# hyunjik11/GPT

Measured on AMD Instinct MI355X. Metric: SGLD steps/sec (kin40k, n_feat=500/dim, r=5), higher is better.
Workload: dtype f64

## Files before the change

gpt_amd/csrc/chain.hip:

```cpp
#include "device_util.h"

namespace gpt {

constexpr int kChainBufs = 1;
constexpr int kChainDMax = 8;
constexpr int kChainTPW8 = 1;
constexpr int kChainTasks = 2;
constexpr int kChainG = 2;
constexpr int kChainQPL = 4;
constexpr int kChainQP = 64 * kChainQPL;
constexpr int kChainRun = 64;
constexpr int kChainRunS = 72;
constexpr int kChainQS = 264;

constexpr int kChainMMax = 256;

GPT_HD constexpr int chain_scratch_dbl(int r, bool own_x1) {
  const int s0a = 7 * 4 * r * r, s0b = 64 * 8;
  return (s0a > s0b ? s0a : s0b) + (own_x1 ? 7 : 2) * r * r + 3 * r * r + r;
}
GPT_HD constexpr int al16c(int x) { return (x + 15) & ~15; }

template <int R, int G, int WV = kChainDMax>
struct ChainLds {
  static constexpr int DRG = kChainDMax * R * G;
  static constexpr int TS = 2 * (DRG + G);
  static constexpr int NTMAX = kChainQPL * G;
  static constexpr int o_IT = 0;
  static constexpr int o_w = al16c(o_IT + 4 * kChainQP * kChainDMax);
  static constexpr int o_y = al16c(o_w + 8 * kChainQP);
  static constexpr int o_temp = al16c(o_y + 8 * kChainMMax);
  static constexpr int o_fp = al16c(o_temp + 8 * 2 * TS);
  static constexpr int o_gwp = al16c(o_fp + 8 * kChainQPL * G);
  static constexpr int o_misc = al16c(o_gwp + 8 * NTMAX * 64);
  static constexpr int o_touch = al16c(o_misc + 8 * 16);
  static constexpr int o_un = al16c(o_touch + 256);
  static constexpr int L_dbl = G * kChainQS + WV * G * R * kChainRunS;
  static constexpr bool own_x1 = WV == kChainDMax;
  static constexpr int x_dbl = chain_scratch_dbl(R, own_x1);
  static constexpr int o_tab = al16c(o_un + 8 * (L_dbl > x_dbl * WV ? L_dbl : x_dbl * WV));
  static constexpr bool tab = WV == kChainDMax;
  static constexpr int bytes = al16c(o_tab + (tab ? 8 * 64 : 0));
};

#ifndef CHAIN_TIMELINE
#define CHAIN_TIMELINE 2
#endif

#ifndef CHAIN_SSTAMP
#define CHAIN_SSTAMP 0
#endif
#ifndef CHAIN_STAMPS
#define CHAIN_STAMPS CHAIN_SSTAMP
#endif
#define CHAIN_FENCE() do {} while (0)
#ifndef CHAIN_PRIO
#define CHAIN_PRIO 2
#endif
#define CHAIN_SETPRIO(hi_upper)                                                             \
  do {                                                                                      \
    if (CHAIN_PRIO) {                                                                       \
      if ((k >= 4) == (hi_upper)) __builtin_amdgcn_s_setprio(1);                            \
      else __builtin_amdgcn_s_setprio(0);                                                   \
    }                                                                                       \
  } while (0)
#if !CHAIN_STAMPS
#define CSTAMP(slot) CHAIN_FENCE()
#endif
#if CHAIN_TIMELINE
#define TSTAMP_ANY(i)                                                                       \
  do {                                                                                      \
    if (P.tline && tid == 0 && (i) < kTimelineSteps + 2) {                                  \
      long long* ts_ = P.tline + (size_t)blockIdx.x * kTimeline + 2 * (i);                  \
      ts_[0] = (long long)__builtin_amdgcn_s_memrealtime();                                \
      ts_[1] = (long long)__builtin_amdgcn_s_memtime();                                    \
    }                                                                                       \
  } while (0)
#else
#define TSTAMP_ANY(i) do {} while (0)
#endif
#if CHAIN_TIMELINE == 1
#define TSTAMP(i) TSTAMP_ANY(i)
#else
#define TSTAMP(i) do {} while (0)
#endif
#if CHAIN_STAMPS
#define CSTAMP(slot)                                                                        \
  do {                                                                                      \
    if (P.stamps && tid == 0)                                                               \
      P.stamps[(size_t)blockIdx.x * kStamps + (slot)] = (long long)__builtin_amdgcn_s_memtime(); \
  } while (0)
#endif

#if CHAIN_STAMPS
#define LSTAMP(slot)                                                                        \
  do {                                                                                      \
    if (P.stamps && g0 == 20 && lane == 0 && (k == 0 || k == 4))                            \
      P.stamps[(size_t)(gridDim.x + blockIdx.x) * kStamps + (k ? 8 : 0) + (slot)] =         \
          (long long)__builtin_amdgcn_s_memtime();                                         \
  } while (0)
#else
#define LSTAMP(slot) CHAIN_FENCE()
#endif

#define SSTAMP(slot)                                                                        \
  do {                                                                                      \
    if ((slot) == 4) CHAIN_SETPRIO(false);        \
    if ((slot) == 7) CHAIN_SETPRIO(true);        \
    if (CHAIN_SSTAMP && P.stamps && lane == 0 && (k == 0 || k == 4))                                        \
      P.stamps[(size_t)((2 + (slot) / 8) * gridDim.x + blockIdx.x) * kStamps + (k ? 8 : 0) + \
               (slot) % 8] = (long long)__builtin_amdgcn_s_memtime();                       \
  } while (0)

template <int J>
__device__ __forceinline__ bool row_in(int jj, int j, int n) {
  return (J >= 2 && jj < J / 2) || j < n;
}

__device__ __forceinline__ void lds_barrier() {
  asm volatile("s_waitcnt lgkmcnt(0)\n\ts_barrier" ::: "memory");
}

template <int R, int J, int G, int WV>
__global__ __launch_bounds__(64 * WV, WV == 4 ? 2 : 1) void chain_kernel(StepParams P,
                                                                const ChainDesc* chains,
                                                                const long long* __restrict__ tbase,
                                                                int t_local, int nsteps) {
  extern __shared__ __attribute__((aligned(16))) unsigned char smem[];
  __shared__ __attribute__((aligned(16))) double pbuf[kChainBufs * WV * G * 64 * J];
  __shared__ __attribute__((aligned(16))) int ibuf[2 * kChainMMax];
  const ChainDesc* Cp = chains + blockIdx.x;
  const int tid = threadIdx.x, lane = tid & 63, k = uni(tid >> 6);
  const int n = P.n, D = P.D, Q = P.Q, m = P.m, NTH = 64 * D;
  using L = ChainLds<R, G, WV>;
  const int NCH = (Q + 63) / 64, NT = NCH * G;
  int* IT_l = (int*)(smem + L::o_IT);
  double* w_l = (double*)(smem + L::o_w);
  int* idx_l = ibuf;
  double* y_l = (double*)(smem + L::o_y);
  double* temp_l = (double*)(smem + L::o_temp);
  double* fp_l = (double*)(smem + L::o_fp);
  double* gwp_l = (double*)(smem + L::o_gwp);
  double* misc = (double*)(smem + L::o_misc);
  int* flag = (int*)(misc + 8);
  double* wVr = (double*)(smem + L::o_un);
  double* X = (double*)(smem + L::o_un) + k * L::x_dbl;
  double* xi_l = X;
  double* pw0 = pbuf + k * (kChainBufs * G * 64 * J);
  [[maybe_unused]] double* bscr = wVr + G * kChainQS + k * G * R * kChainRunS;

  TSTAMP_ANY(0);
#if CHAIN_TIMELINE
  if (P.tline && tid == 0) {
    long long* ts_ = P.tline + (size_t)blockIdx.x * kTimeline + kTimeline - 2;
    ts_[0] = (long long)__builtin_amdgcn_s_getreg((31 << 11) | 4);
    ts_[1] = (long long)__builtin_amdgcn_s_getreg((31 << 11) | 20);
  }
#endif
  const long long t0 = tbase[0] + t_local;
  if (t0 >= P.total_steps) return;
  if (__hip_atomic_load(Cp->status, __ATOMIC_RELAXED, __HIP_MEMORY_SCOPE_AGENT) != 0) return;
  CSTAMP(0);
  const long long tend = min(P.total_steps, t0 + (long long)nsteps);

  auto batch_at = [&](const int32_t* order, int ep_, int bb_, int& bt) -> const int32_t* {
    bt = min(m, P.N - bb_ * m);
    return order + (size_t)ep_ * P.N + (size_t)bb_ * m;
  };
  auto next_pos = [&](int& ep_, int& bb_) {
    if (++bb_ == P.nb) { bb_ = 0; ep_ ^= 1; }
  };
  long long t = t0;
  int ep, bb;
  {
    const int ee = (int)(t0 / P.nb);
    bb = (int)(t0 - (long long)ee * P.nb);
    ep = ee & 1;
  }
  int st_cd;
  long long st_slot;
  {
    const long long post0 = t0 - P.burnin_steps;
    long long cd;
    if (post0 < 0) {
      cd = P.store_every - 1 - post0;
      st_slot = 0;
    } else {
      const long long rem = (post0 + 1) % P.store_every;
      cd = rem ? P.store_every - rem : 0;
      st_slot = (post0 + 1 + cd) / P.store_every - 1;
    }
    st_cd = (int)min(cd, (long long)0x7fffffff);
  }
  int Bt;
  const int32_t* ord = batch_at(Cp->order, ep, bb, Bt);
  const long long koff = (long long)n * k, rstride = (long long)n * D;
  const double* phi_k = uni_ptr(Cp->phi) + koff;
  auto stage_rows = [&](const int (&rows)[G], int ln, double* pw) {
#pragma unroll
    for (int gg = 0; gg < G; ++gg) {
      const char* rb = (const char*)(phi_k + (long long)rows[gg] * rstride);
      __attribute__((address_space(3))) double* dst =
          (__attribute__((address_space(3))) double*)(pw + gg * 64 * J);
      if constexpr (J >= 2) {
#pragma unroll
        for (int s = 0; s < J / 2; ++s) {
          const unsigned o = min(16u * ln + 1024u * s, 8u * n - 16u);
          __builtin_amdgcn_global_load_lds((const __attribute__((address_space(1))) void*)(rb + o),
                                           (__attribute__((address_space(3))) void*)(dst + 128 * s),
                                           16, 0, 0);
        }
      } else {
#pragma unroll
        for (int s = 0; s < 2; ++s) {
          const unsigned o = min(4u * ln + 256u * s, 8u * n - 4u);
          __builtin_amdgcn_global_load_lds((const __attribute__((address_space(1))) void*)(rb + o),
                                           (__attribute__((address_space(3))) void*)(dst + 32 * s),
                                           4, 0, 0);
        }
      }
    }
  };
  auto stage = [&](int g0n, int ln, double* pw) {
    int rows[G];
#pragma unroll
    for (int gg = 0; gg < G; ++gg) rows[gg] = uni(idx_l[min(g0n + gg, Bt - 1)]);
    stage_rows(rows, ln, pw);
  };
  {
    int rows0[G];
#pragma unroll
    for (int gg = 0; gg < G; ++gg) rows0[gg] = gptr(ord)[min(gg, Bt - 1)];
    stage_rows(rows0, lane, pw0);
  }

  constexpr int DRG = L::DRG;
  {
    for (int o = tid; o < Q * kChainDMax; o += NTH) {
      const int kk = o / Q, q = o - kk * Q;
      IT_l[o] = kk < D ? (kk * R + gptr(P.I0)[q + Q * kk]) * G : DRG;
    }
    for (int o = tid; o < G; o += NTH) wVr[o * kChainQS + kChainQP] = 0.0;
    for (int o = tid; o < 2 * G; o += NTH) {
      temp_l[o / G * L::TS + DRG + o % G] = 1.0;
      temp_l[o / G * L::TS + 2 * DRG + G + o % G] = 1.0;
    }
    for (int o = tid; o < kChainQPL * G; o += NTH) fp_l[o] = 0.0;
  }
  if constexpr (L::tab) sincos_tab_fill((double*)(smem + L::o_tab), tid, NTH);
  for (int q = tid; q < Q; q += NTH) w_l[q] = gptr(Cp->w)[(size_t)(t0 & 1) * Q + q];
  if (tid == 0) flag[0] = 0;
  {
    const double* yv = Cp->y;
    int* i0_l = ibuf + ((int)t0 & 1) * kChainMMax;
    for (int i = tid; i < Bt; i += NTH) {
      const int row = gptr(ord)[i];
      i0_l[i] = row;
      y_l[i] = gptr(yv)[row];
    }
    if (t0 + 1 < tend) {
      int e1 = ep, b1 = bb, B1;
      next_pos(e1, b1);
      const int32_t* ord1 = batch_at(Cp->order, e1, b1, B1);
      int* i1_l = ibuf + ((int)(t0 + 1) & 1) * kChainMMax;
      for (int i = tid; i < B1; i += NTH) i1_l[i] = gptr(ord1)[i];
    }
  }
  double u[J][R];
  {
    const double* Ug = Cp->U + (size_t)n * R * k;
#pragma unroll
    for (int jj = 0; jj < J; ++jj) {
      const int j = lane + 64 * jj;
      const int jc = min(j, n - 1);
#pragma unroll
      for (int l = 0; l < R; ++l) {
        const double x = gptr(Ug + (size_t)n * l)[jc];
        u[jj][l] = j < n ? x : 0.0;
      }
    }
  }
  __syncthreads();
  CSTAMP(1);
  TSTAMP_ANY(1);



  constexpr int TPW = (J >= 8 && WV > 4) ? kChainTPW8 : kChainTasks;
  for (;;) {
  const int lane = lane_id(), tid = 64 * k + lane;
  idx_l = ibuf + ((int)t & 1) * kChainMMax;
  for (int o = tid; o < G; o += NTH) wVr[o * kChainQS + kChainQP] = 0.0;
  unsigned itp[TPW][kChainDMax / 4];
#pragma unroll
  for (int x = 0; x < TPW; ++x) {
    const int task = k + D * x;
    const int c = task < NT ? task % NCH : 0;
    const int qq = min(64 * c + lane, Q - 1);
#pragma unroll
    for (int h = 0; h < kChainDMax / 4; ++h) {
      unsigned v = 0;
#pragma unroll
      for (int b4 = 0; b4 < 4; ++b4) v |= (unsigned)IT_l[(4 * h + b4) * Q + qq] << (8 * b4);
      itp[x][h] = v;
    }
  }
  unsigned gq[4];
  {
    const int rl0 = min(lane >> 3, R - 1), rs0 = lane & 7;
    const int32_t* rq = P.runq + ((size_t)k * R + rl0) * kChainRun + rs0;
#pragma unroll
    for (int i = 0; i < 4; ++i)
      gq[i] = (unsigned)gptr(rq)[16 * i] | ((unsigned)gptr(rq)[16 * i + 8] << 16);
  }
  double acc[J][R];
#pragma unroll
  for (int jj = 0; jj < J; ++jj)
#pragma unroll
    for (int l = 0; l < R; ++l) acc[jj][l] = 0.0;
  double vsave[TPW], gw[TPW];
#pragma unroll
  for (int x = 0; x < TPW; ++x) { vsave[x] = 0.0; gw[x] = 0.0; }

  int slot = 0;
  for (int g0 = 0; g0 < Bt; g0 += G, slot ^= 1) {
    int ln = lane;
    asm volatile("" : "+v"(ln));
    LSTAMP(0);
    asm volatile("s_waitcnt vmcnt(0)" ::: "memory");
    LSTAMP(1);
    double* pw = pw0;
    double p[G][J];
#pragma unroll
    for (int gg = 0; gg < G; ++gg)
#pragma unroll
      for (int jj = 0; jj < J; ++jj)
        p[gg][jj] = pw[gg * 64 * J + ln + 64 * jj];
    asm volatile("s_waitcnt lgkmcnt(0)" ::: "memory");
    LSTAMP(2);
    double* tsl = temp_l + slot * L::TS;
    const int rl = min(ln >> 3, R - 1);
    {
      double v[G * R];
#pragma unroll
      for (int x = 0; x < G * R; ++x) v[x] = 0.0;
#pragma unroll
      for (int gg = 0; gg < G; ++gg)
#pragma unroll
        for (int jj = 0; jj < J; ++jj)
#pragma unroll
          for (int l = 0; l < R; ++l) v[gg * R + l] = fma(p[gg][jj], u[jj][l], v[gg * R + l]);
      obf_run<G * R, G * R>(v, ln);
      int vi;
      bool wr;
      obf_index<G * R>(ln, vi, wr);
      if (wr) {
        const int gg = vi / R, l = vi - gg * R;
        tsl[(k * R + l) * G + gg] = v[0];
        tsl[DRG + G + (k * R + l) * G + gg] = rcp_nr(v[0]);
      }
    }
    if (g0 + G < Bt) stage(g0 + G, ln, pw);
    LSTAMP(3);
    lds_barrier();
    LSTAMP(4);
#pragma unroll
    for (int x = 0; x < TPW; ++x) {
      const int task = k + D * x;
      if (task >= NT) break;
      const int gg = task / NCH, c = task - gg * NCH;
      const int q = 64 * c + ln;
      const bool ok = q < Q;
      const double wq = w_l[min(q, Q - 1)];
      double tv[kChainDMax];
#pragma unroll
      for (int kk = 0; kk < kChainDMax; ++kk)
        tv[kk] = tsl[((itp[x][kk >> 2] >> (8 * (kk & 3))) & 0xff) + gg];
      static_assert(kChainDMax == 8, "product tree below is written for 8 dimensions");
      const double V = ((tv[0] * tv[1]) * (tv[2] * tv[3])) * ((tv[4] * tv[5]) * (tv[6] * tv[7]));
      const double wV = ok ? wq * V : 0.0;
      if (ok) wVr[gg * kChainQS + q] = wV;
      vsave[x] = ok ? V : 0.0;
      const double fs = wave_sum(wV);
      if (lane == 0) fp_l[gg * kChainQPL + c] = fs;
    }
    LSTAMP(5);
    lds_barrier();
    LSTAMP(6);
    double res[G];
#pragma unroll
    for (int gg = 0; gg < G; ++gg) {
      double f = fp_l[gg * kChainQPL];
#pragma unroll
      for (int c = 1; c < kChainQPL; ++c) f += fp_l[gg * kChainQPL + c];
      res[gg] = (g0 + gg < Bt) ? y_l[g0 + gg] - f : 0.0;
    }
#pragma unroll
    for (int gg = 0; gg < G; ++gg) {
      const double* wr = wVr + gg * kChainQS;
      double a = wr[gq[0] & 0xffff];
#pragma unroll
      for (int i = 1; i < 8; ++i) a += wr[(gq[i >> 1] >> (16 * (i & 1))) & 0xffff];
      a = (group8_sum(a) * tsl[DRG + G + (k * R + rl) * G + gg]) * res[gg];
      double cc[R];
#pragma unroll
      for (int l = 0; l < R; ++l) cc[l] = readlane_d(a, 8 * l);
#pragma unroll
      for (int jj = 0; jj < J; ++jj) {
        const double pv = p[gg][jj];
#pragma unroll
        for (int l = 0; l < R; ++l) acc[jj][l] = fma(pv, cc[l], acc[jj][l]);
      }
    }
#pragma unroll
    for (int x = 0; x < TPW; ++x) {
      const int task = k + D * x;
      if (task >= NT) break;
      const int gg = task / NCH;
      double rr = res[0];
#pragma unroll
      for (int g2 = 1; g2 < G; ++g2) if (gg == g2) rr = res[g2];
      gw[x] = fma(vsave[x], rr, gw[x]);
    }
    LSTAMP(7);
  }
  CSTAMP(2);

  const ChainDesc* Cq = Cp;
  asm volatile("" : "+s"(Cq));
  ChainDesc C;
  {
    const auto* Cc = cptr(Cq);
    C.y = Cc->y; C.order = Cc->order; C.w = Cc->w; C.U = Cc->U;
    C.w_store = Cc->w_store; C.U_store = Cc->U_store; C.diag = Cc->diag; C.status = Cc->status;
    C.seed = Cc->seed; C.epsw = Cc->epsw; C.epsU = Cc->epsU; C.signal_var = Cc->signal_var;
    C.sigma_w = Cc->sigma_w;
  }
  int Nn = P.N;
  asm volatile("" : "+s"(Nn));
  const double cN = (double)Nn / (double)Bt;
  const bool store = st_cd == 0;
  const long long slot_s = store ? st_slot : 0;

#pragma unroll
  for (int x = 0; x < TPW; ++x) {
    const int task = k + D * x;
    if (task >= NT) break;
    gwp_l[task * 64 + lane] = gw[x];
  }
  SSTAMP(0);
  __syncthreads();
  SSTAMP(1);
  CHAIN_SETPRIO(true);
  int ep1 = ep, bb1 = bb, Bn = 0;
  next_pos(ep1, bb1);
  const int* idx_n = ibuf + ((int)(t + 1) & 1) * kChainMMax;
  double y_n = 0.0;
  if (t + 1 < tend) {
    Bn = min(m, P.N - bb1 * m);
    y_n = gptr(C.y)[idx_n[min(tid, Bn - 1)]];
  }
  {
    const double inv_sw2 = 1.0 / (C.sigma_w * C.sigma_w);
    const double sqe = sqrt(C.epsw);
    double gn2 = 0.0;
#pragma unroll 1
    for (int q = tid; q < Q; q += NTH) {
      const int c = q >> 6, ln = q & 63;
      double g = 0.0;
      for (int gg = 0; gg < G; ++gg) g += gwp_l[(gg * NCH + c) * 64 + ln];
      const double wq = w_l[q];
      const double gradw = cN * g / C.signal_var - wq * inv_sw2;
      double step = C.epsw * gradw / 2;
      step += sqe * normal_at(C.seed, (uint32_t)q, (uint32_t)t, kWNoise, 0);
      const double wn = wq + step;
      w_l[q] = wn;
      if (t + 1 == tend) gptr_w(C.w)[(size_t)((t + 1) & 1) * Q + q] = wn;
      if (store && C.w_store) gptr_w(C.w_store)[(size_t)slot_s * Q + q] = wn;
      gn2 = fma(gradw, gradw, gn2);
    }
    if (C.diag) {
      gn2 = wave_sum(gn2);
      if (lane == 0) misc[k] = gn2;
    }
  }
  SSTAMP(2);
  asm volatile("" : "+v"(y_n));
  if (t + 1 < tend) {
    y_l[min(tid, Bn - 1)] = y_n;
    for (int i = tid + NTH; i < Bn; i += NTH) y_l[i] = gptr(C.y)[idx_n[i]];
    int rows0[G];
#pragma unroll
    for (int gg = 0; gg < G; ++gg) rows0[gg] = uni(idx_n[min(gg, Bn - 1)]);
    stage_rows(rows0, lane, pw0);
    if (t + 2 < tend) {
      int ep2 = ep1, bb2 = bb1, B2;
      next_pos(ep2, bb2);
      const int32_t* ord2 = batch_at(C.order, ep2, bb2, B2);
#pragma unroll
      for (int x = 0; x < kChainMMax / 64; ++x) {
        const int c0 = 64 * k + x * NTH;
        if (c0 < B2)
          __builtin_amdgcn_global_load_lds(
              (const __attribute__((address_space(1))) void*)(ord2 + min(c0 + lane, B2 - 1)),
              (__attribute__((address_space(3))) void*)(idx_l + c0), 4, 0, 0);
      }
    }
  }
  CSTAMP(3);
  SSTAMP(3);

  const double cU = cN / C.signal_var;
  const double sq = sqrt(C.epsU);
  double gu2 = 0.0;
  {
    constexpr int NQJ = (J + 3) / 4;
    constexpr int NZ = J >= 4 ? 4 : 2;
    const int NQ = unoise_nq(n);
#pragma unroll 1
    for (int l = 0; l < R; ++l) {
#pragma unroll
      for (int q = 0; q < NQJ; ++q) {
        double z[4];
        if constexpr (L::tab)
          normal_quad_tab<NZ>(C.seed, (uint32_t)((l * NQ + q) * 64 + lane), (uint32_t)t, kUNoise,
                              (uint32_t)k, (const double*)(smem + L::o_tab), z);
        else
          normal_quad<NZ>(C.seed, (uint32_t)((l * NQ + q) * 64 + lane), (uint32_t)t, kUNoise,
                          (uint32_t)k, z);
#pragma unroll
        for (int i = 0; i < NZ; ++i)
          if (4 * q + i < J) xi_l[(4 * q + i) * 64 + lane] = z[i];
      }
#pragma unroll
      for (int L = 0; L < R; ++L) {
        if (l == L) {
          double xv[J];
#pragma unroll
          for (int jj = 0; jj < J; ++jj) xv[jj] = xi_l[jj * 64 + lane];
#pragma unroll
          for (int jj = 0; jj < J; ++jj) {
            const bool in = row_in<J>(jj, lane + 64 * jj, n);
            const double Gv = in ? acc[jj][L] * cU : 0.0;
            gu2 = fma(Gv, Gv, gu2);
            acc[jj][L] = in ? sq * Gv / 2 + xv[jj] : 0.0;
          }
        }
      }
    }
  }
  if (C.diag) {
    gu2 = wave_sum(gu2);
    if (lane == 0) C.diag[(size_t)t * (1 + D) + 1 + k] = sqrt(gu2);
  }
  CSTAMP(4);
  SSTAMP(4);
  {
    constexpr int NN = 2 * R;
    constexpr int S0 = (7 * NN * NN > 64 * 8) ? 7 * NN * NN : 64 * 8;
    constexpr bool kOwnX1 = L::own_x1;
    double* X0 = X;
    double* Ec = X + S0;
    double* X1 = kOwnX1 ? X + S0 : X0;
    double* Mg = X + S0 + (kOwnX1 ? 7 * R * R : NN * R);
    double* Ag = Mg + R * R;
    double* Sg = Ag + R * R;
    double* nr = Sg + R * R;
    wave_sync();
#pragma unroll
    for (int a = 0; a < R; ++a) {
      double v[R];
#pragma unroll
      for (int bb = 0; bb < R; ++bb) {
        double s0 = 0.0;
#pragma unroll
        for (int jj = 0; jj < J; ++jj) s0 = fma(u[jj][a], acc[jj][bb], s0);
        v[bb] = s0;
      }
      wave_sum_to_lds<R>(v, Mg + a * R);
    }
    wave_sync();
    SSTAMP(5);
#pragma unroll
    for (int bb = 0; bb < R; ++bb) {
      double ms[R];
#pragma unroll
      for (int a = 0; a < R; ++a) ms[a] = Mg[a * R + bb] + Mg[bb * R + a];
#pragma unroll
      for (int jj = 0; jj < J; ++jj) {
        double s = 0.0;
#pragma unroll
        for (int a = 0; a < R; ++a) s = fma(u[jj][a], ms[a], s);
        acc[jj][bb] = acc[jj][bb] - s / 2;
      }
    }
      CSTAMP(5);
      SSTAMP(6);
      {
#pragma unroll
        for (int a = 0; a < R; ++a) {
          double v[R];
#pragma unroll
          for (int bb = 0; bb < R; ++bb) {
            double s1 = 0.0;
            if (bb >= a)
#pragma unroll
              for (int jj = 0; jj < J; ++jj) s1 = fma(acc[jj][a], acc[jj][bb], s1);
            v[bb] = s1;
          }
          wave_sum_to_lds<R>(v, Sg + a * R);
        }
      }
      wave_sync();
      const double tt = sq;
      for (int o = lane; o < NN * NN; o += 64) {
        const int i = o / NN, j = o - i * NN;
        const int ia = i < R ? i : i - R, ja = j < R ? j : j - R;
        const double a = (Mg[ia * R + ja] - Mg[ja * R + ia]) / 2;
        double v;
        if (i < R) v = j < R ? a : -Sg[ia <= ja ? ia * R + ja : ja * R + ia];
        else v = j < R ? (ia == j ? 1.0 : 0.0) : a;
        X0[o] = tt * v;
        if (kOwnX1 && i < R && j < R) X1[ia * R + ja] = -tt * a;
        if (!kOwnX1 && i < R && j < R) Ag[ia * R + ja] = a;
      }
      wave_sync();
      long long* xst = (CHAIN_SSTAMP && P.stamps && k == 0)
                           ? P.stamps + (size_t)(4 * gridDim.x + blockIdx.x) * kStamps : nullptr;
      const bool bad = wave_expm<NN>(X0, xst);
      SSTAMP(7);
      if constexpr (!kOwnX1) {
        for (int o = lane; o < NN * R; o += 64) {
          const int a = o / R, l = o - a * R;
          Ec[o] = X0[NN * NN + a * NN + l];
        }
        wave_sync();
        for (int o = lane; o < R * R; o += 64) X1[o] = -tt * Ag[o];
        wave_sync();
      }
      wave_expm<R>(X1, xst ? xst + (size_t)gridDim.x * kStamps : nullptr);
      if (bad && lane == 0) flag[0] = 1;
      CSTAMP(6);
      SSTAMP(8);
      const double* mx = X1 + R * R;
      double* F = Mg;
      const double* El = kOwnX1 ? X0 + NN * NN : Ec;
      constexpr int ES = kOwnX1 ? NN : R;
      wave_sync();
      for (int o = lane; o < NN * R; o += 64) {
        const int a = o / R, l = o - a * R;
        double s = 0.0;
#pragma unroll
        for (int c2 = 0; c2 < R; ++c2) s = fma(El[a * ES + c2], mx[c2 * R + l], s);
        F[o] = s;
      }
      wave_sync();
      SSTAMP(9);
      {
        double Fh[R * R];
#pragma unroll
        for (int x = 0; x < R * R; ++x) Fh[x] = F[x];
#pragma unroll
        for (int jj = 0; jj < J; ++jj) {
          double o[R];
#pragma unroll
          for (int l = 0; l < R; ++l) o[l] = 0.0;
#pragma unroll
          for (int a = 0; a < R; ++a)
#pragma unroll
            for (int l = 0; l < R; ++l) o[l] = fma(u[jj][a], Fh[a * R + l], o[l]);
#pragma unroll
          for (int l = 0; l < R; ++l) u[jj][l] = o[l];
        }
      }
      SSTAMP(10);
      double nrm[R];
#pragma unroll
      for (int l = 0; l < R; ++l) nrm[l] = 0.0;
      {
        double Fh[R * R];
#pragma unroll
        for (int x = 0; x < R * R; ++x) Fh[x] = F[R * R + x];
#pragma unroll
        for (int jj = 0; jj < J; ++jj) {
#pragma unroll
          for (int a = 0; a < R; ++a)
#pragma unroll
            for (int l = 0; l < R; ++l) u[jj][l] = fma(acc[jj][a], Fh[a * R + l], u[jj][l]);
#pragma unroll
          for (int l = 0; l < R; ++l) nrm[l] = fma(u[jj][l], u[jj][l], nrm[l]);
        }
      }
      SSTAMP(11);
      wave_sum_to_lds<R>(nrm, nr);
      wave_sync();
      SSTAMP(12);
#pragma unroll
      for (int l = 0; l < R; ++l) {
        const double isc = 1.0 / sqrt(nr[l]);
#pragma unroll
        for (int jj = 0; jj < J; ++jj) u[jj][l] = u[jj][l] * isc;
      }
    }
    SSTAMP(13);
    if (CHAIN_PRIO) __builtin_amdgcn_s_setprio(0);
    if (CHAIN_STAMPS && P.stamps && lane == 0)
    P.stamps[(size_t)blockIdx.x * kStamps + 8 + k] = (long long)__builtin_amdgcn_s_memtime();
  __syncthreads();
    if (C.diag && tid == 0) {
      double s = 0.0;
      for (int w2 = 0; w2 < D; ++w2) s += misc[w2];
      C.diag[(size_t)t * (1 + D)] = sqrt(s);
    }
    if (flag[0]) {
      if (tid == 0) __hip_atomic_store(C.status, 1, __ATOMIC_RELAXED, __HIP_MEMORY_SCOPE_AGENT);
      return;
    }
    double* Uk = uni_ptr((t + 1 == tend) ? C.U + (size_t)n * R * k : nullptr);
    double* Us =
        uni_ptr((store && C.U_store) ? C.U_store + ((size_t)slot_s * D + k) * n * R : nullptr);
    if (Uk || Us) {
#pragma unroll
      for (int jj = 0; jj < J; ++jj) {
        const int j = lane + 64 * jj;
        if (row_in<J>(jj, j, n))
#pragma unroll
          for (int l = 0; l < R; ++l) {
            if (Uk) gptr_w(Uk)[j + (size_t)n * l] = u[jj][l];
            if (Us) gptr_w(Us)[j + (size_t)n * l] = u[jj][l];
          }
      }
    }
    CSTAMP(7);
    SSTAMP(15);
    TSTAMP(2 + (int)(t - t0));
    if (store) { st_cd = P.store_every - 1; ++st_slot; } else --st_cd;
    if (++t >= tend) break;
    ep = ep1;
    bb = bb1;
    Bt = Bn;
  }
#if CHAIN_TIMELINE == 2
  TSTAMP_ANY(2 + (int)(tend - 1 - t0));
#endif
}

static_assert(contains(ChainWVs{}, kChainDMax), "the wide U phase has one wave per dimension");

static int chain_wv(int D) { return D <= 4 ? 4 : kChainDMax; }
static size_t chain_static_lds(int J, int WV) {
  return 8 * (size_t)kChainBufs * WV * kChainG * 64 * J + 2 * 4 * kChainMMax;
}

static int chain_J(int n) { return n <= 64 ? 1 : (n <= 128 ? 2 : (n <= 256 ? 4 : (n <= 512 ? 8 : 0))); }

size_t chain_lds_bytes(int n, int D, int r, int Q, int m) {
  (void)n; (void)Q; (void)m;
  return with_value_or(ChainRanks{}, r, (size_t)1 << 30, [&](auto R) {
    return with_value_or(ChainWVs{}, chain_wv(D), (size_t)1 << 30, [&](auto WV) {
      return (size_t)ChainLds<R, kChainG, WV>::bytes;
    });
  });
}

bool chain_supported(int n, int D, int r, int Q, int m, bool langevin, bool stiefel, int max_run) {
  if (max_run > kChainRun) return false;
  if (!langevin || !stiefel) return false;
  if (D < 1 || D > kChainDMax || r < 1 || r > 5 || chain_J(n) == 0) return false;
  if (chain_J(n) >= 2 && (n & 1)) return false;
  if (Q > kChainQP || m > kChainMMax) return false;
  const int NT = (Q + 63) / 64 * kChainG;
  if (NT > ((chain_J(n) >= 8 && D > 4) ? kChainTPW8 : kChainTasks) * D) return false;
  return chain_lds_bytes(n, D, r, Q, m) + chain_static_lds(chain_J(n), chain_wv(D)) <= 160 * 1024;
}

hipError_t launch_chain(const StepParams& P, const ChainDesc* chains, int nchains,
                        const long long* tbase, int t_local, int nsteps, hipStream_t st) {
  const int J = chain_J(P.n);
  const size_t lds = chain_lds_bytes(P.n, P.D, P.r, P.Q, P.m);
  dim3 grid(nchains), block(64 * P.D);
  return with_value(ChainRanks{}, P.r, [&](auto R) {
    return with_value(ChainJs{}, J, [&](auto JJ) {
      return with_value(ChainWVs{}, chain_wv(P.D), [&](auto WV) {
        return launch_big_lds<chain_kernel<R, JJ, kChainG, WV>>(
            (int)(kMaxLds - chain_static_lds(JJ, WV)), grid, block, lds, st, P, chains, tbase,
            t_local, nsteps);
      });
    });
  });
}

}
```

Before: 3.187 million.

## Double-buffer the batch staging ring for J=8 chains and reuse it as scratch

For the J=8, eight-wave configuration, the per-wave staging buffer becomes a two-slot ring. Data for group g0+2G is prefetched while group g0 is processed, and the loop waits on a partial vmcnt rather than draining all outstanding loads. The post-batch X scratch is placed in the second ring slot so total LDS stays within budget, and an unused run-scratch region is removed. This adds LDS pressure and more outstanding global loads, plus extra waits at loop exit and early return.

```diff
diff --git a/gpt_amd/csrc/chain.hip b/gpt_amd/csrc/chain.hip
--- a/gpt_amd/csrc/chain.hip
+++ b/gpt_amd/csrc/chain.hip
@@ -2,15 +2,14 @@
 
 namespace gpt {
 
-constexpr int kChainBufs = 1;
 constexpr int kChainDMax = 8;
+GPT_HD constexpr int chain_bufs(int J, int WV) { return (J == 8 && WV == kChainDMax) ? 2 : 1; }
 constexpr int kChainTPW8 = 1;
 constexpr int kChainTasks = 2;
 constexpr int kChainG = 2;
 constexpr int kChainQPL = 4;
 constexpr int kChainQP = 64 * kChainQPL;
 constexpr int kChainRun = 64;
-constexpr int kChainRunS = 72;
 constexpr int kChainQS = 264;
 
 constexpr int kChainMMax = 256;
@@ -21,7 +20,7 @@
 }
 GPT_HD constexpr int al16c(int x) { return (x + 15) & ~15; }
 
-template <int R, int G, int WV = kChainDMax>
+template <int R, int G, int WV = kChainDMax, int BUFS = 1>
 struct ChainLds {
   static constexpr int DRG = kChainDMax * R * G;
   static constexpr int TS = 2 * (DRG + G);
@@ -35,10 +34,12 @@
   static constexpr int o_misc = al16c(o_gwp + 8 * NTMAX * 64);
   static constexpr int o_touch = al16c(o_misc + 8 * 16);
   static constexpr int o_un = al16c(o_touch + 256);
-  static constexpr int L_dbl = G * kChainQS + WV * G * R * kChainRunS;
+  static constexpr bool x_in_ring = BUFS == 2;
+  static constexpr int L_dbl = G * kChainQS;
   static constexpr bool own_x1 = WV == kChainDMax;
   static constexpr int x_dbl = chain_scratch_dbl(R, own_x1);
-  static constexpr int o_tab = al16c(o_un + 8 * (L_dbl > x_dbl * WV ? L_dbl : x_dbl * WV));
+  static constexpr int un_dbl = (x_in_ring || L_dbl > x_dbl * WV) ? L_dbl : x_dbl * WV;
+  static constexpr int o_tab = al16c(o_un + 8 * un_dbl);
   static constexpr bool tab = WV == kChainDMax;
   static constexpr int bytes = al16c(o_tab + (tab ? 8 * 64 : 0));
 };
@@ -121,18 +122,31 @@
   asm volatile("s_waitcnt lgkmcnt(0)\n\ts_barrier" ::: "memory");
 }
 
+template <int N>
+__device__ __forceinline__ void wait_vm() {
+  static_assert(N >= 0 && N < 64, "vmcnt is a 6-bit counter");
+  asm volatile("" ::: "memory");
+  __builtin_amdgcn_s_waitcnt((N & 15) | ((N >> 4) << 14) | (7 << 4) | (15 << 8));
+  asm volatile("" ::: "memory");
+}
+
 template <int R, int J, int G, int WV>
 __global__ __launch_bounds__(64 * WV, WV == 4 ? 2 : 1) void chain_kernel(StepParams P,
                                                                 const ChainDesc* chains,
                                                                 const long long* __restrict__ tbase,
                                                                 int t_local, int nsteps) {
   extern __shared__ __attribute__((aligned(16))) unsigned char smem[];
-  __shared__ __attribute__((aligned(16))) double pbuf[kChainBufs * WV * G * 64 * J];
+  constexpr bool kRing = chain_bufs(J, WV) == 2;
+  constexpr int PW = G * 64 * J;
+  constexpr int ND = G * (J >= 2 ? J / 2 : 2);
+  __shared__ __attribute__((aligned(16))) double pbufA[WV * PW];
+  __shared__ __attribute__((aligned(16))) double pbufB[kRing ? WV * PW : 2];
   __shared__ __attribute__((aligned(16))) int ibuf[2 * kChainMMax];
   const ChainDesc* Cp = chains + blockIdx.x;
   const int tid = threadIdx.x, lane = tid & 63, k = uni(tid >> 6);
   const int n = P.n, D = P.D, Q = P.Q, m = P.m, NTH = 64 * D;
-  using L = ChainLds<R, G, WV>;
+  using L = ChainLds<R, G, WV, chain_bufs(J, WV)>;
+  static_assert(!L::x_in_ring || L::x_dbl <= PW, "the post-batch scratch fits the wave's slice");
   const int NCH = (Q + 63) / 64, NT = NCH * G;
   int* IT_l = (int*)(smem + L::o_IT);
   double* w_l = (double*)(smem + L::o_w);
@@ -144,10 +158,15 @@
   double* misc = (double*)(smem + L::o_misc);
   int* flag = (int*)(misc + 8);
   double* wVr = (double*)(smem + L::o_un);
-  double* X = (double*)(smem + L::o_un) + k * L::x_dbl;
+  double* pw0 = pbufA + k * PW;
+  [[maybe_unused]] double* pw1 = pbufB + (kRing ? k * PW : 0);
+  double* X = L::x_in_ring ? pw1 : (double*)(smem + L::o_un) + k * L::x_dbl;
+  if constexpr (L::x_in_ring) {
+    auto* x3 = (__attribute__((address_space(3))) double*)X;
+    asm volatile("" : "+s"(x3));
+    X = (double*)x3;
+  }
   double* xi_l = X;
-  double* pw0 = pbuf + k * (kChainBufs * G * 64 * J);
-  [[maybe_unused]] double* bscr = wVr + G * kChainQS + k * G * R * kChainRunS;
 
   TSTAMP_ANY(0);
 #if CHAIN_TIMELINE
@@ -322,14 +341,34 @@
 #pragma unroll
   for (int x = 0; x < TPW; ++x) { vsave[x] = 0.0; gw[x] = 0.0; }
 
+  if constexpr (kRing) {
+#pragma unroll
+    for (int i = 0; i < 4; ++i) asm volatile("" : "+v"(gq[i]));
+    if (Bt > G) {
+      int ln = lane;
+      asm volatile("" : "+v"(ln));
+      stage(G, ln, pw1);
+    }
+  }
+
   int slot = 0;
   for (int g0 = 0; g0 < Bt; g0 += G, slot ^= 1) {
     int ln = lane;
     asm volatile("" : "+v"(ln));
     LSTAMP(0);
-    asm volatile("s_waitcnt vmcnt(0)" ::: "memory");
+    if constexpr (kRing) {
+      if (g0 + G < Bt) wait_vm<ND>();
+      else wait_vm<0>();
+    } else {
+      asm volatile("s_waitcnt vmcnt(0)" ::: "memory");
+    }
     LSTAMP(1);
     double* pw = pw0;
+    if constexpr (kRing) {
+      auto* q = (__attribute__((address_space(3))) double*)(slot ? pw1 : pw0);
+      asm volatile("" : "+s"(q));
+      pw = (double*)q;
+    }
     double p[G][J];
 #pragma unroll
     for (int gg = 0; gg < G; ++gg)
@@ -338,6 +377,9 @@
         p[gg][jj] = pw[gg * 64 * J + ln + 64 * jj];
     asm volatile("s_waitcnt lgkmcnt(0)" ::: "memory");
     LSTAMP(2);
+    if constexpr (kRing) {
+      if (g0 + 2 * G < Bt) stage(g0 + 2 * G, ln, pw);
+    }
     double* tsl = temp_l + slot * L::TS;
     const int rl = min(ln >> 3, R - 1);
     {
@@ -360,7 +402,9 @@
         tsl[DRG + G + (k * R + l) * G + gg] = rcp_nr(v[0]);
       }
     }
-    if (g0 + G < Bt) stage(g0 + G, ln, pw);
+    if constexpr (!kRing) {
+      if (g0 + G < Bt) stage(g0 + G, ln, pw);
+    }
     LSTAMP(3);
     lds_barrier();
     LSTAMP(4);
@@ -424,6 +468,7 @@
     }
     LSTAMP(7);
   }
+  if constexpr (kRing) wait_vm<0>();
   CSTAMP(2);
 
   const ChainDesc* Cq = Cp;
@@ -714,6 +759,7 @@
     }
     if (flag[0]) {
       if (tid == 0) __hip_atomic_store(C.status, 1, __ATOMIC_RELAXED, __HIP_MEMORY_SCOPE_AGENT);
+      if constexpr (kRing) wait_vm<0>();
       return;
     }
     double* Uk = uni_ptr((t + 1 == tend) ? C.U + (size_t)n * R * k : nullptr);
@@ -749,16 +795,17 @@
 
 static int chain_wv(int D) { return D <= 4 ? 4 : kChainDMax; }
 static size_t chain_static_lds(int J, int WV) {
-  return 8 * (size_t)kChainBufs * WV * kChainG * 64 * J + 2 * 4 * kChainMMax;
+  return 8 * (size_t)chain_bufs(J, WV) * WV * kChainG * 64 * J + 2 * 4 * kChainMMax;
 }
 
 static int chain_J(int n) { return n <= 64 ? 1 : (n <= 128 ? 2 : (n <= 256 ? 4 : (n <= 512 ? 8 : 0))); }
 
 size_t chain_lds_bytes(int n, int D, int r, int Q, int m) {
-  (void)n; (void)Q; (void)m;
+  (void)Q; (void)m;
   return with_value_or(ChainRanks{}, r, (size_t)1 << 30, [&](auto R) {
     return with_value_or(ChainWVs{}, chain_wv(D), (size_t)1 << 30, [&](auto WV) {
-      return (size_t)ChainLds<R, kChainG, WV>::bytes;
+      return chain_bufs(chain_J(n), WV) == 2 ? (size_t)ChainLds<R, kChainG, WV, 2>::bytes
+                                             : (size_t)ChainLds<R, kChainG, WV, 1>::bytes;
     });
   });
 }
```

Result: faster. 3.241 million, median of 6 (+1.7%).
